# C-bowman/inference-tools

Measured on AMD Instinct MI355X. Metric: GpRegressor fit+predict wall-time and GFLOP/s at N=16384, d=8; % fp64 MFMA peak, higher is better.
Workload: dtype f64

## Files before the change

inference-tools_amd/csrc/api.hip:

```cpp
#include "api_internal.h"
#include <malloc.h>


thread_local std::string g_create_err;


int lane_streams(gpmi_ctx* c, Lane& L) {
  const size_t index = c->lanes.size() - 1;
  L.owns_stream = index < 2;
  if (!L.owns_stream) L.stream = c->lanes[index % 2].stream;
  if (L.owns_stream) HIPCHK(c, hipStreamCreateWithFlags(&L.stream, hipStreamNonBlocking));
  hipDeviceProp_t prop;
  HIPCHK(c, hipGetDeviceProperties(&prop, c->device));
  c->ncu = prop.multiProcessorCount;
  HIPCHK(c, hipEventCreateWithFlags(&L.ev_la, hipEventDisableTiming));
  HIPCHK(c, hipEventCreateWithFlags(&L.ev_panel, hipEventDisableTiming));
  HIPCHK(c, hipEventCreateWithFlags(&L.ev_join, hipEventDisableTiming));
  HIPCHK(c, hipEventCreateWithFlags(&L.ev_main, hipEventDisableTiming));
  HIPCHK(c, hipEventCreateWithFlags(&L.ev_slice, hipEventDisableTiming));
  return GPMI_OK;
}


bool ensure_masked_pair(gpmi_ctx* c, Lane& L, int k) {
// ... 305 lines not shown
  L.early.ident = early_identity;
  L.early.ident_ld = c->ld;
  L.identity_ready = false;
  if (!early_fill) L.early.pending = false;
  potrf_lower(c, L, L.A, c->np, c->ld, L.invD, L.info + slot, allow_lookahead);
  if (!early_fill) L.early.pending = true;
  lane_run_early(L, s);
  if (prebuild_inv2 && L.su[0] && c->np >= 4 * GPMI_OB) {
    HIPCHK(c, hipEventRecord(L.ev_join, s));
    HIPCHK(c, hipStreamWaitEvent(L.su[0], L.ev_join, 0));
    if (int rc = ensure_inv2(c, L, L.su[0])) return rc;
    HIPCHK(c, hipEventRecord(L.ev_main, L.su[0]));
  }
  trsv_forward(c, s, L.A, c->np, c->ld, L.invD, L.vec + 2 * c->np, L.vec, L.info + slot, BatchShape(), true);
  if (prebuild_inv2 && L.inv2_valid && L.su[0]) {
    HIPCHK(c, hipEventRecord(L.ev_la, s));
    HIPCHK(c, hipStreamWaitEvent(L.su[0], L.ev_la, 0));
    launch_lml_reduce(L.su[0], L.vec, L.A, c->ld, c->np, L.red + 2 * slot);
    HIPCHK(c, hipEventRecord(L.ev_main, L.su[0]));
  } else {
    launch_lml_reduce(s, L.vec, L.A, c->ld, c->np, L.red + 2 * slot);
  }
  HIPCHK(c, hipGetLastError());
  return GPMI_OK;
}

int ensure_second_matrix(gpmi_ctx* c, Lane& L) {
  if (!L.B2) HIPCHK(c, hipMalloc(&L.B2, sizeof(double) * c->np * c->ld));
  return GPMI_OK;
}

int ensure_inv2(gpmi_ctx* c, Lane& F, hipStream_t s) {
  if (F.inv2_valid) return GPMI_OK;
  const int64_t nob = (c->np / GPMI_NB + 3) / 4;
  if (!F.inv2) HIPCHK(c, hipMalloc(&F.inv2, sizeof(double) * nob * GPMI_OB * GPMI_OB));
  if (!F.inv2_t) HIPCHK(c, hipMalloc(&F.inv2_t, sizeof(double) * nob * 256 * 256));
  build_inv2(s, F.A, c->np, c->ld, F.invD, F.inv2, F.inv2_t);
  HIPCHK(c, hipGetLastError());
  F.inv2_valid = true;
  return GPMI_OK;
}

int ensure_trsm_panel(gpmi_ctx* c, int64_t rows) {
  if (rows <= c->trsm_panel_rows) return GPMI_OK;
  if (c->trsm_panel) (void)hipFree(c->trsm_panel);
  c->trsm_panel = nullptr;
  c->trsm_panel_rows = 0;
  HIPCHK(c, hipMalloc(&c->trsm_panel, sizeof(double) * rows * (GPMI_OB + 32)));
  c->trsm_panel_rows = rows;
  return GPMI_OK;
}

int enqueue_inverse_factor(gpmi_ctx* c, Lane& L, Lane& F) {
  if (int rc = ensure_inv2(c, F, L.stream)) return rc;
  if (int rc = ensure_trsm_panel(c, c->np)) return rc;
  if (!L.identity_ready) launch_set_identity(L.stream, L.B2, c->ld, c->np);
  L.identity_ready = false;
  trsm_rows_forward(c, L.stream, F.A, c->np, c->ld, F.inv2, L.B2, c->np, true, nullptr, c->trsm_panel);
  return GPMI_OK;
}

int ensure_batch_ws(gpmi_ctx* c, int want) {
  const int64_t per = c->np * c->ld * (int64_t)sizeof(double);
  static const int64_t budget_gib = [] {
    const char* e = std::getenv("GPMI_BATCH_GIB");
    const int v = e ? std::atoi(e) : 24;
    return (int64_t)(v >= 1 && v <= 200 ? v : 24);
  }();
  static const int max_chunk = [] {
    const char* e = std::getenv("GPMI_BATCH_MAX");
    const int v = e ? std::atoi(e) : 512;
    return v >= 2 && v <= 4096 ? v : 512;
  }();
  int cap = (int)((budget_gib << 30) / per);
  if (cap > max_chunk) cap = max_chunk;
  if (cap < 1) cap = 1;
  if (want > cap) want = cap;
  if (want <= c->bcap) return GPMI_OK;
  ARGCHK(c, c->bpend[0] == 0 && c->bpend[1] == 0,
         "the batch workspace cannot grow while an asynchronous batch is pending (gpmi_lml_batch_wait first)");
  auto fr = [](double*& p) {
// ... 569 lines not shown
```

inference-tools_amd/csrc/api_linv.hip:

```cpp
#include "api_internal.h"

void linv_free(LinvState& S) {
  for (double** p : {&S.A, &S.At, &S.y, &S.sig2, &S.zero, &S.K, &S.T, &S.J, &S.J2, &S.Q, &S.X, &S.invD, &S.inv2,
                     &S.inv2_t, &S.panel, &S.vec, &S.gws}) {
    if (*p) (void)hipFree(*p);
    *p = nullptr;
  }
  S = LinvState();
}

namespace {

__global__ void linv_add_diag_kernel(double* __restrict__ J, int64_t ld, const double* __restrict__ sig2,
                                     int64_t mp) {
  const int64_t i = (int64_t)blockIdx.x * blockDim.x + threadIdx.x;
  if (i < mp) J[i * ld + i] += sig2[i];
}


int linv_alloc(gpmi_ctx* c, double** p, int64_t doubles) {
  if (*p) return GPMI_OK;
  HIPCHK(c, hipMalloc(p, sizeof(double) * doubles));
  ZERO_SYNC(c, *p, sizeof(double) * doubles);
  return GPMI_OK;
// ... 95 lines not shown
  *lml = -0.5 * L.h_red[0] - L.h_red[1];
  INFOCHK(c, L.h_info[0]);
  if (info) *info = L.h_info[0];
  return GPMI_OK;
}

int gpmi_linv_lml(gpmi_ctx* c, int kernel, const double* theta, int n_theta, double extra_diag,
                  const double* mu, double* lml, int* info) {
  if (!c) return GPMI_ERR_ARG;
  if (int rc = linv_ready(c)) return rc;
  KParams p;
  if (int rc = make_params(c, kernel, theta, n_theta, extra_diag, p)) return rc;
  return linv_lml_impl(c, p, nullptr, mu, lml, info);
}

int gpmi_linv_lml_dense(gpmi_ctx* c, const double* K_host, const double* mu, double* lml, int* info) {
  if (!c) return GPMI_ERR_ARG;
  if (int rc = linv_ready(c)) return rc;
  ARGCHK(c, K_host, "K is NULL");
  return linv_lml_impl(c, KParams{}, K_host, mu, lml, info);
}

static int linv_lml_grad_impl(gpmi_ctx* c, const KParams& p, int n_theta, const double* K_host, const double* mu,
                              double* lml, double* grad_theta, double* trace_q, double* G_host, double* at_alpha,
                              int* info) {
  ARGCHK(c, mu && lml && (grad_theta || G_host), "mu / lml / output is NULL");
  if (int rc = set_device(c)) return rc;
  LinvState& S = c->linv;
  Lane& L = c->lanes[0];
  hipStream_t s = L.stream;
  const int nt = (int)(c->np / GPMI_NB), mt = (int)(S.mp / GPMI_NB);
  const int64_t vmax = S.mp > c->np ? S.mp : c->np;
  if (int rc = linv_alloc(c, &S.J2, S.mp * S.ldm)) return rc;
  if (int rc = linv_alloc(c, &S.inv2, (int64_t)((mt + 3) / 4) * GPMI_OB * GPMI_OB)) return rc;
  if (int rc = linv_alloc(c, &S.inv2_t, (int64_t)((mt + 3) / 4) * 256 * 256)) return rc;
  if (int rc = linv_alloc(c, &S.panel, S.mp * (GPMI_OB + 32))) return rc;
  const int64_t need = n_theta >= 0 ? grad_ws_doubles(c->np, n_theta) : 0;
  if (S.gws_doubles < need) {
    if (S.gws) (void)hipFree(S.gws);
    S.gws = nullptr;
    S.gws_doubles = 0;
    HIPCHK(c, hipMalloc(&S.gws, sizeof(double) * need));
    S.gws_doubles = need;
  }
  if (int rc = linv_factor(c, p, mu, K_host)) return rc;
  double* v = S.vec;
  double* alpha = S.vec + 4 * vmax;
  double* w = S.vec + 5 * vmax;
  double* gout = L.red + 16;
  trsv_backward(c, s, S.J, S.mp, S.ldm, S.invD, v, alpha, L.info);
  launch_rows_dot(s, S.At, S.ldm, c->np, S.mp, alpha, w);
  build_inv2(s, S.J, S.mp, S.ldm, S.invD, S.inv2, S.inv2_t);
  launch_set_identity(s, S.J2, S.ldm, S.mp);
  trsm_rows_forward(c, s, S.J, S.mp, S.ldm, S.inv2, S.J2, S.mp, true, nullptr, S.panel);
  launch_gemm(s, TILES_LOWER, OP_ASSIGN, false, 1, S.J, S.ldm, S.J2, S.ldm, S.J2, S.ldm, mt, mt, (int)S.mp);
  launch_mirror_lower(s, S.J, S.ldm, S.mp);
  launch_gemm_nt(s, TILES_RECT, OP_ASSIGN, S.T, c->ld, S.J, S.ldm, S.At, S.ldm, mt, nt, (int)S.mp);
  launch_gemm(s, TILES_RECT, OP_ASSIGN, true, 0, S.K, c->ld, S.At, S.ldm, S.T, c->ld, nt, nt, (int)S.mp);
  if (n_theta >= 0) launch_lml_grad(s, p, n_theta, c->x, c->n, c->np, S.K, c->ld, w, w, S.gws, gout);
  HIPCHK(c, hipGetLastError());
  HIPCHK(c, hipMemcpyAsync(L.h_red, L.red, 2 * sizeof(double), hipMemcpyDeviceToHost, s));
  if (n_theta >= 0)
    HIPCHK(c, hipMemcpyAsync(L.h_red + 16, gout, sizeof(double) * (n_theta + 1), hipMemcpyDeviceToHost, s));
  if (G_host)
    HIPCHK(c, hipMemcpy2DAsync(G_host, sizeof(double) * c->n, S.K, sizeof(double) * c->ld, sizeof(double) * c->n, c->n,
                               hipMemcpyDeviceToHost, s));
  HIPCHK(c, hipMemcpyAsync(L.h_info, L.info, sizeof(int), hipMemcpyDeviceToHost, s));
  if (at_alpha) HIPCHK(c, hipMemcpyAsync(at_alpha, w, sizeof(double) * c->n, hipMemcpyDeviceToHost, s));
  HIPCHK(c, hipStreamSynchronize(s));
// ... 6 lines not shown
  return GPMI_OK;
}

int gpmi_linv_lml_grad(gpmi_ctx* c, int kernel, const double* theta, int n_theta, double extra_diag,
                       const double* mu, double* lml, double* grad_theta, double* trace_q,
                       double* at_alpha, int* info) {
  if (!c) return GPMI_ERR_ARG;
  if (int rc = linv_ready(c)) return rc;
  KParams p;
  if (int rc = make_params(c, kernel, theta, n_theta, extra_diag, p)) return rc;
  ARGCHK(c, grad_theta, "grad_theta is NULL");
  return linv_lml_grad_impl(c, p, n_theta, nullptr, mu, lml, grad_theta, trace_q, nullptr, at_alpha, info);
}

int gpmi_linv_lml_grad_dense(gpmi_ctx* c, const double* K_host, const double* mu, double* lml, double* G_host,
                             double* at_alpha, int* info) {
  if (!c) return GPMI_ERR_ARG;
  if (int rc = linv_ready(c)) return rc;
  ARGCHK(c, K_host && G_host, "K / G is NULL");
  return linv_lml_grad_impl(c, KParams{}, -1, K_host, mu, lml, nullptr, nullptr, G_host, at_alpha, info);
}

static int linv_posterior_impl(gpmi_ctx* c, const KParams& p, const double* K_host, const double* mu, double* mean,
                               double* cov, int* info) {
  ARGCHK(c, mu && mean, "mu / mean is NULL");
  if (int rc = set_device(c)) return rc;
  LinvState& S = c->linv;
  Lane& L = c->lanes[0];
  hipStream_t s = L.stream;
  const int nt = (int)(c->np / GPMI_NB), mt = (int)(S.mp / GPMI_NB);
  const int64_t vmax = S.mp > c->np ? S.mp : c->np;
  if (int rc = linv_alloc(c, &S.Q, c->np * S.ldm)) return rc;
  if (int rc = linv_alloc(c, &S.X, c->np * S.ldm)) return rc;
  if (int rc = linv_alloc(c, &S.inv2, (int64_t)((mt + 3) / 4) * GPMI_OB * GPMI_OB)) return rc;
  if (int rc = linv_alloc(c, &S.inv2_t, (int64_t)((mt + 3) / 4) * 256 * 256)) return rc;
  if (int rc = linv_factor(c, p, mu, K_host)) return rc;
  double* v = S.vec;
  double* dm = S.vec + 5 * vmax;
  build_inv2(s, S.J, S.mp, S.ldm, S.invD, S.inv2, S.inv2_t);
  launch_gemm_nt(s, TILES_RECT, OP_ASSIGN, S.Q, S.ldm, S.K, c->ld, S.A, c->ld, nt, mt, (int)c->np);
  trsm_rows_forward(c, s, S.J, S.mp, S.ldm, S.inv2, S.Q, c->np, false, S.X, nullptr);
  launch_rows_dot(s, S.X, S.ldm, c->np, S.mp, v, dm);
  if (cov) launch_gemm_nt(s, TILES_RECT, OP_SUB, S.K, c->ld, S.X, S.ldm, S.X, S.ldm, nt, nt, (int)S.mp);
  HIPCHK(c, hipGetLastError());
  HIPCHK(c, hipMemcpyAsync(L.h_info, L.info, sizeof(int), hipMemcpyDeviceToHost, s));
  HIPCHK(c, hipMemcpyAsync(mean, dm, sizeof(double) * c->n, hipMemcpyDeviceToHost, s));
  if (cov)
    HIPCHK(c, hipMemcpy2DAsync(cov, sizeof(double) * c->n, S.K, sizeof(double) * c->ld, sizeof(double) * c->n,
                               c->n, hipMemcpyDeviceToHost, s));
  HIPCHK(c, hipStreamSynchronize(s));
  c->fitted = false;
  for (int64_t i = 0; i < c->n; ++i) mean[i] += mu[i];
  INFOCHK(c, L.h_info[0]);
  if (info) *info = L.h_info[0];
  return GPMI_OK;
}

int gpmi_linv_posterior(gpmi_ctx* c, int kernel, const double* theta, int n_theta, double extra_diag,
                        const double* mu, double* mean, double* cov, int* info) {
  if (!c) return GPMI_ERR_ARG;
  if (int rc = linv_ready(c)) return rc;
  KParams p;
  if (int rc = make_params(c, kernel, theta, n_theta, extra_diag, p)) return rc;
  return linv_posterior_impl(c, p, nullptr, mu, mean, cov, info);
}

int gpmi_linv_posterior_dense(gpmi_ctx* c, const double* K_host, const double* mu, double* mean, double* cov,
                              int* info) {
// ... 9 lines not shown
```

inference-tools_amd/csrc/gemm_f64.hip:

```cpp
#include <cstdlib>

#include "gemm_tiles.h"

namespace {

using namespace gemm_tiles;

struct GemmArgs {
  double* C;
  const double* A;
  const double* B;
  int64_t ldc, lda, ldb;
  int ntr, ntc, k;
  int kskip;
  unsigned long long* stamp;
  int64_t sC, sA, sB;
  int split, tile_base;
  FlowHook hook;
  int zlocal_tiles;
  int mixed_full;
};

struct WgId {
  int wid;
// ... 237 lines not shown
                      int64_t ldc, const double* A, int64_t lda, const double* B, int64_t ldb, int ntr,
                      int ntc, int k, unsigned long long* stamp, const GemmBatch& bt, int part, int64_t nfull,
                      int64_t nend = -1) {
  if (ntr <= 0 || ntc <= 0 || k <= 0) return;
  if (tiles == TILES_LOWER && ntc > ntr) ntc = ntr;
  const int64_t big = (tiles == TILES_RECT) ? (int64_t)ntr * ntc
                                            : (int64_t)ntc * (ntc + 1) / 2 + (int64_t)(ntr - ntc) * ntc;
  int bm = 128, bn = 128;
  static const int64_t BIG_MIN = [] {
    const char* e = std::getenv("GPMI_BIG_MIN");
    return (int64_t)(e ? std::atoi(e) : 384);
  }();
  static const int64_t SMALL_M32_MAX = [] {
    const char* e = std::getenv("GPMI_M32_MAX");
    return (int64_t)(e ? std::atoi(e) : 192);
  }();
  const int64_t m32_max = bt.ncu_hint > 0 ? SMALL_M32_MAX * bt.ncu_hint / 256 : SMALL_M32_MAX;
  const bool small = part == 0 && ((k <= 128) || (big * bt.count < BIG_MIN));
  if (part == 2) {
    bm = 64;
    bn = 64;
  } else if (small && kskip != 1) {
    if (ntc == 1 && tiles == TILES_RECT && op == OP_ASSIGN) {
      bm = (!b_kmajor && (int64_t)ntr * 2 * bt.count <= m32_max) ? 32 : 64;
    } else if (!b_kmajor || op == OP_SUB) {
      bm = 64;
      bn = 64;
      if (tiles == TILES_RECT && !b_kmajor && k > 128 && big * 4 * bt.count <= m32_max && !bt.ring_order_only) bm = 32;
      static const bool bn32 = [] {
        const char* e = std::getenv("GPMI_CHAIN_BN32");
        return !e || std::atoi(e) != 0;
      }();
      if (bn32 && bm == 32 && kskip == 2 && op == OP_ASSIGN && big * 8 * bt.count <= 2 * 256) bn = 32;
    }
  }
  if (part == 0 && kskip == 4 && b_kmajor && op == OP_ASSIGN && tiles == TILES_RECT) {
    if (big * 16 * bt.count <= 2 * 256) {
      bm = 32;
      bn = 32;
    } else {
      bm = 64;
      bn = 128;
    }
  }
  if (bt.b_lower_tri && kskip == 0 && bn == 128 && bm <= 64 && ntc == 1 && k == 128 && !b_kmajor && op == OP_ASSIGN) kskip = 3;
  GemmArgs g{C, A, B, ldc, lda, ldb, ntr * (128 / bm), ntc * (128 / bn), k, kskip, stamp,
             bt.sC, bt.sA, bt.sB, part == 2 ? 1 : 0, (part == 2 || part == 3) ? (int)nfull : 0, bt.hook, 0, 0};
  int64_t nwg;
  if (tiles == TILES_RECT)
    nwg = (int64_t)g.ntr * g.ntc;
  else
    nwg = (int64_t)g.ntc * (g.ntc + 1) / 2 + (int64_t)(g.ntr - g.ntc) * g.ntc;
  if (part == 1) nwg = nfull;
  if (nend < 0 || nend > big) nend = big;
  if (part == 2) nwg = 4 * (nend - nfull);
  if (part == 3) nwg = nend - nfull;
  if (part == 4) {
    g.mixed_full = (int)nfull;
    nwg = nfull + 4 * (nend - nfull);
  }
  if (nwg <= 0) return;
  dim3 grid((unsigned)nwg, 1, (unsigned)bt.count), block(256);
  static const bool batch_xcd = [] {
    const char* e = std::getenv("GPMI_BATCH_XCD");
    return !e || std::atoi(e) != 0;
  }();
// ... 61 lines not shown
    if (b_kmajor) GPMI_LAUNCH(TILES_RECT, OP_ASSIGN, 1, 32, 32); else GPMI_LAUNCH(TILES_RECT, OP_ASSIGN, 0, 32, 32);
  } else if (bm == 32) {
    if (op == OP_SUB) GPMI_LAUNCH(TILES_RECT, OP_SUB, 0, 32, 64); else GPMI_LAUNCH(TILES_RECT, OP_ASSIGN, 0, 32, 64);
  } else {
    if (tiles == TILES_RECT) {
      if (op == OP_SUB) {
        if (b_kmajor) GPMI_LAUNCH(TILES_RECT, OP_SUB, 1, 64, 64); else GPMI_LAUNCH(TILES_RECT, OP_SUB, 0, 64, 64);
      } else {
        GPMI_LAUNCH(TILES_RECT, OP_ASSIGN, 0, 64, 64);
      }
    } else {
      if (op == OP_SUB) GPMI_LAUNCH(TILES_LOWER, OP_SUB, 0, 64, 64); else GPMI_LAUNCH(TILES_LOWER, OP_ASSIGN, 0, 64, 64);
    }
  }
#undef GPMI_LAUNCH
}
}

void launch_gemm(hipStream_t s, GemmTiles tiles, GemmOp op, bool b_kmajor, int kskip, double* C,
                 int64_t ldc, const double* A, int64_t lda, const double* B, int64_t ldb, int ntr,
                 int ntc, int k, unsigned long long* stamp, const GemmBatch& bt) {
  launch_gemm_part(s, tiles, op, b_kmajor, kskip, C, ldc, A, lda, B, ldb, ntr, ntc, k, stamp, bt, 0, 0);
}

int64_t gemm_split_point(int64_t T, int ncu, int k) {
  static const int64_t BIG_MIN = [] {
    const char* e = std::getenv("GPMI_BIG_MIN");
    return (int64_t)(e ? std::atoi(e) : 384);
  }();
  static const int64_t SPLIT_PCT = [] {
    const char* e = std::getenv("GPMI_SPLIT_PCT");
    return (int64_t)(e ? std::atoi(e) : 70);
  }();
  if (k <= 128 || T < BIG_MIN || ncu <= 0) return T;
  const int64_t rem = T % ncu;
  if (rem == 0 || rem * 100 > (int64_t)ncu * SPLIT_PCT) return T;
  return T - rem;
}

bool gemm_mixed_launches() {
  static const bool mixed = [] {
    const char* e = std::getenv("GPMI_GEMM_MIXED");
    return !e || std::atoi(e) != 0;
  }();
  return mixed;
}

void launch_gemm_nt_split(hipStream_t s, GemmTiles tiles, GemmOp op, double* C, int64_t ldc, const double* A,
                          int64_t lda, const double* B, int64_t ldb, int ntr, int ntc, int k, int64_t nfull,
                          unsigned long long* stamp, unsigned long long* stamp_rest, int64_t nend) {
  if (tiles == TILES_LOWER && ntc > ntr) ntc = ntr;
  const int64_t T = (tiles == TILES_RECT) ? (int64_t)ntr * ntc
                                          : (int64_t)ntc * (ntc + 1) / 2 + (int64_t)(ntr - ntc) * ntc;
  const GemmBatch one{};
  if (nend < 0 || nend > T) nend = T;
  if (nfull >= T) {
    launch_gemm_part(s, tiles, op, false, 0, C, ldc, A, lda, B, ldb, ntr, ntc, k, stamp, one, 0, 0);
    return;
  }
  if (gemm_mixed_launches() && nfull > 0 && nend > nfull && k % 128 == 0 && k > 128) {
    launch_gemm_part(s, tiles, op, false, 0, C, ldc, A, lda, B, ldb, ntr, ntc, k, stamp, one, 4, nfull, nend);
    return;
  }
  launch_gemm_part(s, tiles, op, false, 0, C, ldc, A, lda, B, ldb, ntr, ntc, k, stamp, one, 1, nfull);
  if (nend > nfull)
    launch_gemm_part(s, tiles, op, false, 0, C, ldc, A, lda, B, ldb, ntr, ntc, k, stamp_rest, one, 2, nfull, nend);
}

void launch_gemm_nt_range(hipStream_t s, GemmTiles tiles, GemmOp op, double* C, int64_t ldc, const double* A,
// ... 13 lines not shown
```

inference-tools_amd/csrc/gpmi_internal.h:

```cpp
#pragma once
#include <hip/hip_runtime.h>
#include <cstdint>
#include <string>
#include <vector>

#include "gpmi.h"

constexpr int GPMI_NB = 128;
constexpr int GPMI_MAX_D = 64;
constexpr int GPMI_INFO_FLOW_TIMEOUT = -6;
constexpr int GPMI_NPAIRS = 1;

typedef double d2_t __attribute__((ext_vector_type(2)));
typedef double d4_t __attribute__((ext_vector_type(4)));

static inline int64_t round_up(int64_t v, int64_t m) { return (v + m - 1) / m * m; }

struct KParams {
  int kernel;
  int d;
  double a2;
  double kappa;
  double extra_diag;
  double inv_l2[GPMI_MAX_D];
// ... 263 lines not shown

void launch_gemm(hipStream_t s, GemmTiles tiles, GemmOp op, bool b_kmajor, int kskip, double* C,
                 int64_t ldc, const double* A, int64_t lda, const double* B, int64_t ldb, int ntr,
                 int ntc, int k, unsigned long long* stamp = nullptr, const GemmBatch& bt = GemmBatch());

hipStream_t potrf_first_update_stream(gpmi_ctx* c, Lane& lane, int64_t np, bool allow_lookahead);
void potrf_pair_quiesce(Lane& lane);
void launch_potrf_diag(hipStream_t s, double* Ablk, int64_t ld, double* invD, int* info, int col0,
                       unsigned long long* dbg = nullptr, const BatchShape& bs = BatchShape(), int* pub = nullptr,
                       int pub_val = 0);
void launch_potrf_diag_fault(hipStream_t s, double* Ablk, int64_t ld, const BatchShape& bs = BatchShape());
void potrf_lower_batched(gpmi_ctx* c, hipStream_t s, double* A, int64_t np, int64_t ld, double* invD,
                         int* info, const BatchShape& bs);
void launch_kbuild_square_batched(hipStream_t s, int kernel, const KParams* pdev, int batch, const double* x,
                                  int64_t n, int64_t np, const double* noise, double* A, int64_t ld,
                                  int64_t stride, int d, int64_t noise_stride = 0);
void potrf_lower(gpmi_ctx* c, Lane& lane, double* A, int64_t np, int64_t ld, double* invD,
                 int* info, bool allow_lookahead = true);

bool potrf_flow_enabled(gpmi_ctx* c, Lane& lane, int m);
bool potrf_flow_tail(gpmi_ctx* c, Lane& lane, double* A, int64_t ld, double* invD, int* info, int nt, int t0);
void potrf_flow_free(Lane& lane);

void trsv_forward(gpmi_ctx* c, hipStream_t s, const double* L, int64_t np, int64_t ld,
                  const double* invD, const double* r, double* out, int* err = nullptr,
                  const BatchShape& bs = BatchShape(), bool prefilled = false);
void trsv_backward(gpmi_ctx* c, hipStream_t s, const double* L, int64_t np, int64_t ld,
                   const double* invD, const double* r, double* out, int* err = nullptr,
                   const BatchShape& bs = BatchShape(), bool prefilled = false);
void lane_run_early(Lane& lane, hipStream_t s);
void trsm_identity_batched(hipStream_t s, const double* L, int64_t np, int64_t ld, const double* invD, double* Q,
                           const BatchShape& bs);
constexpr int GPMI_OB = 512;
void build_inv2(hipStream_t s, const double* L, int64_t np, int64_t ld, const double* invD, double* inv2,
                double* tmp);
void trsm_rows_forward(gpmi_ctx* c, hipStream_t s, const double* L, int64_t np, int64_t ld,
                       const double* inv2, double* Q, int64_t mp, bool upper_rhs, double* Qout,
                       double* panel);
void launch_set_identity(hipStream_t s, double* Q, int64_t ld, int64_t np, int batch = 1, int64_t sMat = 0);
void launch_copy(hipStream_t s, const double* src, double* dst, int64_t n);
void launch_copy_rows(hipStream_t s, const double* src, int64_t spitch, double* dst, int64_t dpitch, int64_t width,
                      int64_t height);
void launch_residual(hipStream_t s, const double* y, const double* mu, double mu_const, double* r,
                     int64_t n, int64_t np);
void launch_residual_batched(hipStream_t s, const double* y, const double* mus, const double* mu_consts,
                             double* r, int64_t n, int64_t np, const BatchShape& bs);
void launch_lml_reduce(hipStream_t s, const double* v, const double* L, int64_t ld, int64_t np,
                       double* red, const BatchShape& bs = BatchShape());
void launch_rows_dot(hipStream_t s, const double* Q, int64_t ld, int64_t mp, int64_t np,
                     const double* a, double* out, int batch = 1, int64_t sQ = 0, int64_t sVec = 0);
void launch_rows_sumsq(hipStream_t s, const double* Q, int64_t ld, int64_t mp, int64_t np,
                       double base, double* out, int batch = 1, int64_t sQ = 0, int64_t sVec = 0, double sign = 1.0);

void trsm_rows_backward(gpmi_ctx* c, hipStream_t s, const double* L, int64_t np, int64_t ld,
                        const double* invD, double* Q, int64_t mp, const double* inv2 = nullptr, double* panel = nullptr);

void launch_sd_reduce(hipStream_t s, const KParams& p, const double* x, int64_t n, const double* pts,
                      int64_t m, const double* Kq, int64_t ld, const double* W, int64_t ldw,
                      double scale, double* out);
void launch_grad_rhs(hipStream_t s, const KParams& p, const double* x, int64_t n, int64_t np,
                     const double* pts, int64_t rows_valid, int64_t rows_padded, const double* Kq,
                     int64_t ld, double* G);
void launch_grad_cov(hipStream_t s, const KParams& p, const double* G, int64_t ld, int64_t np,
                     int64_t m, double* cov);
```

inference-tools_amd/csrc/solve.hip:

```cpp
#include <cstdlib>
#include <mutex>

#include "gpmi_internal.h"

namespace {

constexpr int NB = GPMI_NB;

__device__ inline double wave_sum(double v) {
#pragma unroll
  for (int off = 32; off > 0; off >>= 1) v += __shfl_down(v, off, 64);
  return v;
}

constexpr unsigned long long FLOW_SENTINEL = 0xFFF8DEADBEEF0000ull;
constexpr int FLOW_THREADS = 512;
constexpr int FLOW_SPIN_LIMIT = 1 << 22;

__device__ inline double flow_poll(const double* p, int* err, bool& dead) {
  const unsigned long long* q = reinterpret_cast<const unsigned long long*>(p);
  unsigned long long bits = __hip_atomic_load(q, __ATOMIC_RELAXED, __HIP_MEMORY_SCOPE_AGENT);
  int spins = 0;
  while (bits == FLOW_SENTINEL && !dead) {
    __builtin_amdgcn_s_sleep(1);
// ... 215 lines not shown
#pragma unroll
      for (int i = 0; i < 8; ++i) {
        const double x = aj[wave + 64 + 8 * i];
        acc[0] = fma(hb[i][0], x, acc[0]);
        acc[1] = fma(hb[i][1], x, acc[1]);
      }
    }
  }
  part[wave][2 * lane] = acc[0];
  part[wave][2 * lane + 1] = acc[1];
  __syncthreads();
  SWEEP_STAMP(2, step);
  if (tid < NB) {
    double s = 0.0;
#pragma unroll
    for (int g = 0; g < 8; ++g) s += part[g][tid];
    u[tid] = wk - s;
  }
  __syncthreads();
  SWEEP_STAMP(3, step);
  {
    double s = 0.0;
#pragma unroll
    for (int i = 0; i < 32; ++i) s = fma(xi[i], u[rg * 32 + i], s);
    part[4 + rg][col] = s;
    __syncthreads();
    if (tid < NB)
      flow_publish(a + (int64_t)k * NB + tid, (part[4][tid] + part[5][tid]) + (part[6][tid] + part[7][tid]));
    SWEEP_STAMP(4, step);
    SWEEP_STAMP_FLUSH(step);
  }
}

__global__ void inv2_seed_kernel(const double* __restrict__ invD, double* __restrict__ inv2, int nt) {
  const int b = blockIdx.z, r = blockIdx.y, cpair = (blockIdx.x * 64 + threadIdx.x) * 2;
  const int t = r >> 7;
  d2_t v = d2_t{0.0, 0.0};
  if ((cpair >> 7) == t && 4 * b + t < nt)
    v = *reinterpret_cast<const d2_t*>(invD + ((int64_t)(4 * b + t) * NB + (r & 127)) * NB + (cpair & 127));
  *reinterpret_cast<d2_t*>(inv2 + ((int64_t)b * GPMI_OB + r) * GPMI_OB + cpair) = v;
}

__global__ void copy_panel_kernel(const double* __restrict__ src, int64_t lds, double* __restrict__ dst,
                                  int64_t ldd) {
  const int64_t r = blockIdx.y;
  const int c = (blockIdx.x * 64 + threadIdx.x) * 2;
  *reinterpret_cast<d2_t*>(dst + r * ldd + c) = *reinterpret_cast<const d2_t*>(src + r * lds + c);
}

__global__ void set_identity_kernel(double* __restrict__ Q, int64_t ld, int64_t np, int64_t sMat) {
  const int64_t j = ((int64_t)blockIdx.x * blockDim.x + threadIdx.x) * 2;
  const int64_t i = blockIdx.y;
  Q += (int64_t)blockIdx.z * sMat;
  if (j < np)
    *reinterpret_cast<d2_t*>(Q + i * ld + j) = d2_t{j == i ? 1.0 : 0.0, j + 1 == i ? 1.0 : 0.0};
}

__global__ void copy_rows_kernel(const double* __restrict__ src, int64_t spitch, double* __restrict__ dst, int64_t dpitch,
                                 int64_t width) {
  const int64_t j = (int64_t)blockIdx.x * blockDim.x + threadIdx.x;
  if (j < width) dst[(int64_t)blockIdx.y * dpitch + j] = src[(int64_t)blockIdx.y * spitch + j];
}

__global__ void copy_kernel(const double* __restrict__ src, double* __restrict__ dst, int64_t n) {
  const int64_t i = (int64_t)blockIdx.x * blockDim.x + threadIdx.x;
  if (i < n) dst[i] = src[i];
}

__global__ void residual_batched_kernel(const double* __restrict__ y, const double* __restrict__ mus,
                                        const double* __restrict__ mu_consts, double* __restrict__ r,
                                        int64_t n, int64_t np, int64_t sVec) {
  const int64_t i = (int64_t)blockIdx.x * blockDim.x + threadIdx.x;
  if (i >= np) return;
// ... 123 lines not shown
    launch_set_identity(s, e.ident, e.ident_ld, e.np);
    lane.identity_ready = true;
  }
}

void trsv_forward(gpmi_ctx* c, hipStream_t s, const double* L, int64_t np, int64_t ld,
                  const double* invD, const double* r, double* out, int* err, const BatchShape& bs, bool prefilled) {
  const int nt = (int)(np / NB);
  flow_gate_enter(c, s, (int64_t)nt);
  ProfScope ps(c, s, GPMI_PROF_SOLVE, (double)np * np, 4.0 * np * np);
  if (!prefilled)
    hipLaunchKernelGGL(flow_fill_kernel, dim3((unsigned)((np + 255) / 256), 1, (unsigned)bs.count), dim3(256), 0, s,
                       out, np, bs.sVec);
  const unsigned grid = bs.count > 1 ? 8u * (unsigned)nt * (unsigned)((bs.count + 7) / 8) : (unsigned)nt;
  hipLaunchKernelGGL(trsv_fwd_flow_kernel, dim3(grid), dim3(FLOW_THREADS), 0, s, L, ld, invD, r, out, err, bs.sMat,
                     bs.sInv, bs.sVec, nt, bs.count);
  flow_gate_leave(c, s, (int64_t)nt);
}

void trsv_backward(gpmi_ctx* c, hipStream_t s, const double* L, int64_t np, int64_t ld,
                   const double* invD, const double* r, double* out, int* err, const BatchShape& bs, bool prefilled) {
  const int nt = (int)(np / NB);
  flow_gate_enter(c, s, (int64_t)nt);
  ProfScope ps(c, s, GPMI_PROF_SOLVE, (double)np * np, 4.0 * np * np);
  if (!prefilled)
    hipLaunchKernelGGL(flow_fill_kernel, dim3((unsigned)((np + 255) / 256), 1, (unsigned)bs.count), dim3(256), 0, s, out,
                       np, bs.sVec);
  const unsigned grid = bs.count > 1 ? 8u * (unsigned)nt * (unsigned)((bs.count + 7) / 8) : (unsigned)nt;
  hipLaunchKernelGGL(trsv_bwd_flow_kernel, dim3(grid), dim3(FLOW_THREADS), 0, s, L, ld, invD, r, out, err, nt, bs.sMat,
                     bs.sInv, bs.sVec, bs.count);
  flow_gate_leave(c, s, (int64_t)nt);
}

void build_inv2(hipStream_t s, const double* L, int64_t np, int64_t ld, const double* invD, double* inv2,
                double* tmp) {
  const int nt = (int)(np / NB);
  const int nob = (nt + 3) / 4;
  const int64_t slot = (int64_t)GPMI_OB * GPMI_OB, tslot = 256 * 256;
  hipLaunchKernelGGL(inv2_seed_kernel, dim3(GPMI_OB / 2 / 64, GPMI_OB, (unsigned)nob), dim3(64), 0, s, invD, inv2,
                     nt);
  auto offdiag = [&](int r0, int c0, int h2, int h1, int count) {
    if (count <= 0 || h2 <= 0) return;
    const GemmBatch b1{count, tslot, 4 * NB * ld + 4 * NB, slot};
    launch_gemm(s, TILES_RECT, OP_ASSIGN, true, 0, tmp, 256, L + (int64_t)r0 * NB * ld + (int64_t)c0 * NB, ld,
                inv2 + (int64_t)c0 * NB * GPMI_OB + (int64_t)c0 * NB, GPMI_OB, h2, h1, h1 * NB, nullptr, b1);
    const GemmBatch b2{count, slot, slot, tslot};
    launch_gemm(s, TILES_RECT, OP_SUB, true, 0, inv2 + (int64_t)r0 * NB * GPMI_OB + (int64_t)c0 * NB, GPMI_OB,
                inv2 + (int64_t)r0 * NB * GPMI_OB + (int64_t)r0 * NB, GPMI_OB, tmp, 256, h2, h1, h2 * NB, nullptr,
                b2);
  };
  offdiag(1, 0, 1, 1, (nt - 1 + 3) / 4);
  offdiag(3, 2, 1, 1, (nt - 3 + 3) / 4);
  const int full = nt / 4;
  offdiag(2, 0, 2, 2, full);
  if (nt % 4 == 3) {
    const int64_t b = full;
    const GemmBatch one{};
    const double* Lb = L + (b * 4 * NB) * ld + b * 4 * NB;
    double* Xb = inv2 + b * slot;
    double* Tb = tmp + b * tslot;
    launch_gemm(s, TILES_RECT, OP_ASSIGN, true, 0, Tb, 256, Lb + (int64_t)2 * NB * ld, ld, Xb, GPMI_OB, 1, 2, 2 * NB,
                nullptr, one);
    launch_gemm(s, TILES_RECT, OP_SUB, true, 0, Xb + (int64_t)2 * NB * GPMI_OB, GPMI_OB,
                Xb + (int64_t)2 * NB * GPMI_OB + 2 * NB, GPMI_OB, Tb, 256, 1, 2, NB, nullptr, one);
  }
}

void trsm_rows_forward(gpmi_ctx* c, hipStream_t s, const double* L, int64_t np, int64_t ld,
                       const double* inv2, double* Q, int64_t mp, bool upper_rhs, double* Qout,
                       double* panel) {
  const int nt = (int)(np / NB), mt_all = (int)(mp / NB);
  const int OBT = GPMI_OB / NB;
  const int64_t ldp = GPMI_OB + 32;
  ProfScope ps(c, s, GPMI_PROF_TRSM, (double)mp * np * np, 4.0 * np * np);
  for (int J = 0; J < nt; J += OBT) {
    const int Je = (J + OBT < nt) ? J + OBT : nt;
    const int w = Je - J;
    const int mt = upper_rhs ? (Je < mt_all ? Je : mt_all) : mt_all;
    double* QJ = Q + (int64_t)J * NB;
    double* X = Qout ? Qout + (int64_t)J * NB : panel;
    const int64_t ldx = Qout ? ld : ldp;
    launch_gemm(s, TILES_RECT, OP_ASSIGN, false, 2, X, ldx, QJ, ld, inv2 + (int64_t)(J / OBT) * GPMI_OB * GPMI_OB,
                GPMI_OB, mt, w, w * NB);
    const int rest = nt - Je;
    if (rest > 0)
      launch_gemm_nt_split(s, TILES_RECT, OP_SUB, Q + (int64_t)Je * NB, ld, X, ldx,
                           L + (int64_t)Je * NB * ld + (int64_t)J * NB, ld, mt, rest, w * NB,
                           gemm_split_point((int64_t)mt * rest, c->ncu, w * NB));
    if (!Qout) {
      const int64_t rows = (int64_t)mt * NB;
      hipLaunchKernelGGL(copy_panel_kernel, dim3((unsigned)(w * NB / 2 / 64), (unsigned)rows), dim3(64), 0, s, panel,
                         ldp, QJ, ld);
    }
  }
}

void trsm_rows_backward(gpmi_ctx* c, hipStream_t s, const double* L, int64_t np, int64_t ld,
                        const double* invD, double* Q, int64_t mp, const double* inv2, double* panel) {
  const int nt = (int)(np / NB), mt = (int)(mp / NB);
  ProfScope ps(c, s, GPMI_PROF_TRSM, (double)mp * np * np, 4.0 * np * np);
  static const bool wide = [] {
    const char* e = std::getenv("GPMI_BACKWARD_OB");
    return !e || std::atoi(e) != 0;
  }();
  if (wide && inv2 && panel) {
    const int OBT = GPMI_OB / NB;
    const int64_t ldp = GPMI_OB + 32;
    const int nob = (nt + OBT - 1) / OBT;
    for (int b = nob - 1; b >= 0; --b) {
      const int J = b * OBT, Je = (J + OBT < nt) ? J + OBT : nt, w = Je - J;
      double* QJ = Q + (int64_t)J * NB;
      launch_gemm(s, TILES_RECT, OP_ASSIGN, true, 4, panel, ldp, QJ, ld, inv2 + (int64_t)b * GPMI_OB * GPMI_OB, GPMI_OB, mt, w,
                  w * NB);
      if (J > 0)
        launch_gemm(s, TILES_RECT, OP_SUB, true, 0, Q, ld, panel, ldp, L + (int64_t)J * NB * ld, ld, mt, J, w * NB);
      hipLaunchKernelGGL(copy_panel_kernel, dim3((unsigned)(w * NB / 2 / 64), (unsigned)((int64_t)mt * NB)), dim3(64), 0, s, panel,
                         ldp, QJ, ld);
    }
    return;
  }
  for (int k = nt - 1; k >= 0; --k) {
    double* Qk = Q + (int64_t)k * NB;
    launch_gemm(s, TILES_RECT, OP_ASSIGN, true, false, Qk, ld, Qk, ld, invD + (int64_t)k * NB * NB,
                NB, mt, 1, NB);
    if (k > 0)
      launch_gemm(s, TILES_RECT, OP_SUB, true, false, Q, ld, Qk, ld, L + (int64_t)k * NB * ld, ld, mt,
                  k, NB);
  }
}

void launch_set_identity(hipStream_t s, double* Q, int64_t ld, int64_t np, int batch, int64_t sMat) {
  dim3 grid((unsigned)((np / 2 + 255) / 256), (unsigned)np, (unsigned)batch);
  hipLaunchKernelGGL(set_identity_kernel, grid, dim3(256), 0, s, Q, ld, np, sMat);
}

void trsm_identity_batched(hipStream_t s, const double* L, int64_t np, int64_t ld, const double* invD, double* Q,
                           const BatchShape& bs) {
  const int nt = (int)(np / NB);
  const int OBT = 4;
  launch_set_identity(s, Q, ld, np, bs.count, bs.sMat);
  GemmBatch inplace{bs.count, bs.sMat, bs.sMat, bs.sInv};
  inplace.b_lower_tri = true;
  GemmBatch upd{bs.count, bs.sMat, bs.sMat, bs.sMat};
  upd.ring_order_only = true;
  for (int J = 0; J < nt; J += OBT) {
    const int Je = (J + OBT < nt) ? J + OBT : nt;
// ... 58 lines not shown
```

Measured before the change: 55120.

## Widen forward TRSM inverse-block width to 1024 with recursive inv2 build

```diff
diff --git a/inference-tools_amd/csrc/api.hip b/inference-tools_amd/csrc/api.hip
--- a/inference-tools_amd/csrc/api.hip
+++ b/inference-tools_amd/csrc/api.hip
@@ -361,9 +361,8 @@
 
 int ensure_inv2(gpmi_ctx* c, Lane& F, hipStream_t s) {
   if (F.inv2_valid) return GPMI_OK;
-  const int64_t nob = (c->np / GPMI_NB + 3) / 4;
-  if (!F.inv2) HIPCHK(c, hipMalloc(&F.inv2, sizeof(double) * nob * GPMI_OB * GPMI_OB));
-  if (!F.inv2_t) HIPCHK(c, hipMalloc(&F.inv2_t, sizeof(double) * nob * 256 * 256));
+  if (!F.inv2) HIPCHK(c, hipMalloc(&F.inv2, sizeof(double) * inv2_doubles(c->np)));
+  if (!F.inv2_t) HIPCHK(c, hipMalloc(&F.inv2_t, sizeof(double) * inv2_tmp_doubles(c->np)));
   build_inv2(s, F.A, c->np, c->ld, F.invD, F.inv2, F.inv2_t);
   HIPCHK(c, hipGetLastError());
   F.inv2_valid = true;
@@ -375,7 +374,7 @@
   if (c->trsm_panel) (void)hipFree(c->trsm_panel);
   c->trsm_panel = nullptr;
   c->trsm_panel_rows = 0;
-  HIPCHK(c, hipMalloc(&c->trsm_panel, sizeof(double) * rows * (GPMI_OB + 32)));
+  HIPCHK(c, hipMalloc(&c->trsm_panel, sizeof(double) * rows * (predict_ob() + 32)));
   c->trsm_panel_rows = rows;
   return GPMI_OK;
 }
diff --git a/inference-tools_amd/csrc/api_linv.hip b/inference-tools_amd/csrc/api_linv.hip
--- a/inference-tools_amd/csrc/api_linv.hip
+++ b/inference-tools_amd/csrc/api_linv.hip
@@ -151,9 +151,9 @@
   const int nt = (int)(c->np / GPMI_NB), mt = (int)(S.mp / GPMI_NB);
   const int64_t vmax = S.mp > c->np ? S.mp : c->np;
   if (int rc = linv_alloc(c, &S.J2, S.mp * S.ldm)) return rc;
-  if (int rc = linv_alloc(c, &S.inv2, (int64_t)((mt + 3) / 4) * GPMI_OB * GPMI_OB)) return rc;
-  if (int rc = linv_alloc(c, &S.inv2_t, (int64_t)((mt + 3) / 4) * 256 * 256)) return rc;
-  if (int rc = linv_alloc(c, &S.panel, S.mp * (GPMI_OB + 32))) return rc;
+  if (int rc = linv_alloc(c, &S.inv2, inv2_doubles(S.mp))) return rc;
+  if (int rc = linv_alloc(c, &S.inv2_t, inv2_tmp_doubles(S.mp))) return rc;
+  if (int rc = linv_alloc(c, &S.panel, S.mp * (predict_ob() + 32))) return rc;
   const int64_t need = n_theta >= 0 ? grad_ws_doubles(c->np, n_theta) : 0;
   if (S.gws_doubles < need) {
     if (S.gws) (void)hipFree(S.gws);
@@ -226,8 +226,8 @@
   const int64_t vmax = S.mp > c->np ? S.mp : c->np;
   if (int rc = linv_alloc(c, &S.Q, c->np * S.ldm)) return rc;
   if (int rc = linv_alloc(c, &S.X, c->np * S.ldm)) return rc;
-  if (int rc = linv_alloc(c, &S.inv2, (int64_t)((mt + 3) / 4) * GPMI_OB * GPMI_OB)) return rc;
-  if (int rc = linv_alloc(c, &S.inv2_t, (int64_t)((mt + 3) / 4) * 256 * 256)) return rc;
+  if (int rc = linv_alloc(c, &S.inv2, inv2_doubles(S.mp))) return rc;
+  if (int rc = linv_alloc(c, &S.inv2_t, inv2_tmp_doubles(S.mp))) return rc;
   if (int rc = linv_factor(c, p, mu, K_host)) return rc;
   double* v = S.vec;
   double* dm = S.vec + 5 * vmax;
diff --git a/inference-tools_amd/csrc/gemm_f64.hip b/inference-tools_amd/csrc/gemm_f64.hip
--- a/inference-tools_amd/csrc/gemm_f64.hip
+++ b/inference-tools_amd/csrc/gemm_f64.hip
@@ -293,6 +293,15 @@
         return !e || std::atoi(e) != 0;
       }();
       if (bn32 && bm == 32 && kskip == 2 && op == OP_ASSIGN && big * 8 * bt.count <= 2 * 256) bn = 32;
+      static const int wide_wgs = [] {
+        const char* e = std::getenv("GPMI_WIDE_CHAIN_WGS");
+        return e ? std::atoi(e) : 4;
+      }();
+      if (bn32 && tiles == TILES_RECT && !b_kmajor && kskip == 2 && op == OP_ASSIGN && k > GPMI_OB && bt.count == 1 &&
+          !bt.ring_order_only && big * 16 <= (int64_t)wide_wgs * 256) {
+        bm = 32;
+        bn = 32;
+      }
     }
   }
   if (part == 0 && kskip == 4 && b_kmajor && op == OP_ASSIGN && tiles == TILES_RECT) {
@@ -420,9 +429,13 @@
     const char* e = std::getenv("GPMI_SPLIT_PCT");
     return (int64_t)(e ? std::atoi(e) : 70);
   }();
+  static const int64_t SPLIT_PCT_WIDE = [] {
+    const char* e = std::getenv("GPMI_SPLIT_PCT_WIDE");
+    return (int64_t)(e ? std::atoi(e) : 100);
+  }();
   if (k <= 128 || T < BIG_MIN || ncu <= 0) return T;
   const int64_t rem = T % ncu;
-  if (rem == 0 || rem * 100 > (int64_t)ncu * SPLIT_PCT) return T;
+  if (rem == 0 || rem * 100 > (int64_t)ncu * (k > GPMI_OB ? SPLIT_PCT_WIDE : SPLIT_PCT)) return T;
   return T - rem;
 }
 
diff --git a/inference-tools_amd/csrc/gpmi_internal.h b/inference-tools_amd/csrc/gpmi_internal.h
--- a/inference-tools_amd/csrc/gpmi_internal.h
+++ b/inference-tools_amd/csrc/gpmi_internal.h
@@ -319,6 +319,10 @@
 void trsm_identity_batched(hipStream_t s, const double* L, int64_t np, int64_t ld, const double* invD, double* Q,
                            const BatchShape& bs);
 constexpr int GPMI_OB = 512;
+int predict_ob();
+int64_t inv2_doubles(int64_t np);
+int64_t inv2_tmp_doubles(int64_t np);
+const double* inv2_block512(const double* inv2, int b);
 void build_inv2(hipStream_t s, const double* L, int64_t np, int64_t ld, const double* invD, double* inv2,
                 double* tmp);
 void trsm_rows_forward(gpmi_ctx* c, hipStream_t s, const double* L, int64_t np, int64_t ld,
diff --git a/inference-tools_amd/csrc/solve.hip b/inference-tools_amd/csrc/solve.hip
--- a/inference-tools_amd/csrc/solve.hip
+++ b/inference-tools_amd/csrc/solve.hip
@@ -271,13 +271,13 @@
   }
 }
 
-__global__ void inv2_seed_kernel(const double* __restrict__ invD, double* __restrict__ inv2, int nt) {
+__global__ void inv2_seed_kernel(const double* __restrict__ invD, double* __restrict__ inv2, int nt, int pob) {
   const int b = blockIdx.z, r = blockIdx.y, cpair = (blockIdx.x * 64 + threadIdx.x) * 2;
-  const int t = r >> 7;
+  const int t = r >> 7, T = pob >> 7;
   d2_t v = d2_t{0.0, 0.0};
-  if ((cpair >> 7) == t && 4 * b + t < nt)
-    v = *reinterpret_cast<const d2_t*>(invD + ((int64_t)(4 * b + t) * NB + (r & 127)) * NB + (cpair & 127));
-  *reinterpret_cast<d2_t*>(inv2 + ((int64_t)b * GPMI_OB + r) * GPMI_OB + cpair) = v;
+  if ((cpair >> 7) == t && T * b + t < nt)
+    v = *reinterpret_cast<const d2_t*>(invD + ((int64_t)(T * b + t) * NB + (r & 127)) * NB + (cpair & 127));
+  *reinterpret_cast<d2_t*>(inv2 + ((int64_t)b * pob + r) * pob + cpair) = v;
 }
 
 __global__ void copy_panel_kernel(const double* __restrict__ src, int64_t lds, double* __restrict__ dst,
@@ -467,37 +467,56 @@
   flow_gate_leave(c, s, (int64_t)nt);
 }
 
+int predict_ob() {
+  static const int ob = [] {
+    const char* e = std::getenv("GPMI_PREDICT_OB");
+    const int v = e ? std::atoi(e) : 1024;
+    return (v == GPMI_OB || v == 2048) ? v : 1024;
+  }();
+  return ob;
+}
+
+int64_t inv2_doubles(int64_t np) {
+  const int pob = predict_ob(), T = pob / NB;
+  return (int64_t)((np / NB + T - 1) / T) * pob * pob;
+}
+
+int64_t inv2_tmp_doubles(int64_t np) {
+  const int pob = predict_ob(), T = pob / NB;
+  return (int64_t)((np / NB + T - 1) / T) * (pob / 2) * (pob / 2);
+}
+
+const double* inv2_block512(const double* inv2, int b) {
+  const int pob = predict_ob(), r = pob / GPMI_OB;
+  return inv2 + (int64_t)(b / r) * pob * pob + (int64_t)(b % r) * GPMI_OB * (pob + 1);
+}
+
 void build_inv2(hipStream_t s, const double* L, int64_t np, int64_t ld, const double* invD, double* inv2,
                 double* tmp) {
+  const int pob = predict_ob(), T = pob / NB;
   const int nt = (int)(np / NB);
-  const int nob = (nt + 3) / 4;
-  const int64_t slot = (int64_t)GPMI_OB * GPMI_OB, tslot = 256 * 256;
-  hipLaunchKernelGGL(inv2_seed_kernel, dim3(GPMI_OB / 2 / 64, GPMI_OB, (unsigned)nob), dim3(64), 0, s, invD, inv2,
-                     nt);
-  auto offdiag = [&](int r0, int c0, int h2, int h1, int count) {
-    if (count <= 0 || h2 <= 0) return;
-    const GemmBatch b1{count, tslot, 4 * NB * ld + 4 * NB, slot};
-    launch_gemm(s, TILES_RECT, OP_ASSIGN, true, 0, tmp, 256, L + (int64_t)r0 * NB * ld + (int64_t)c0 * NB, ld,
-                inv2 + (int64_t)c0 * NB * GPMI_OB + (int64_t)c0 * NB, GPMI_OB, h2, h1, h1 * NB, nullptr, b1);
-    const GemmBatch b2{count, slot, slot, tslot};
-    launch_gemm(s, TILES_RECT, OP_SUB, true, 0, inv2 + (int64_t)r0 * NB * GPMI_OB + (int64_t)c0 * NB, GPMI_OB,
-                inv2 + (int64_t)r0 * NB * GPMI_OB + (int64_t)r0 * NB, GPMI_OB, tmp, 256, h2, h1, h2 * NB, nullptr,
-                b2);
-  };
-  offdiag(1, 0, 1, 1, (nt - 1 + 3) / 4);
-  offdiag(3, 2, 1, 1, (nt - 3 + 3) / 4);
-  const int full = nt / 4;
-  offdiag(2, 0, 2, 2, full);
-  if (nt % 4 == 3) {
-    const int64_t b = full;
-    const GemmBatch one{};
-    const double* Lb = L + (b * 4 * NB) * ld + b * 4 * NB;
-    double* Xb = inv2 + b * slot;
-    double* Tb = tmp + b * tslot;
-    launch_gemm(s, TILES_RECT, OP_ASSIGN, true, 0, Tb, 256, Lb + (int64_t)2 * NB * ld, ld, Xb, GPMI_OB, 1, 2, 2 * NB,
-                nullptr, one);
-    launch_gemm(s, TILES_RECT, OP_SUB, true, 0, Xb + (int64_t)2 * NB * GPMI_OB, GPMI_OB,
-                Xb + (int64_t)2 * NB * GPMI_OB + 2 * NB, GPMI_OB, Tb, 256, 1, 2, NB, nullptr, one);
+  const int nslot = (nt + T - 1) / T;
+  const int64_t slot = (int64_t)pob * pob, slotL = (int64_t)T * NB * (ld + 1);
+  hipLaunchKernelGGL(inv2_seed_kernel, dim3(pob / 2 / 64, pob, (unsigned)nslot), dim3(64), 0, s, invD, inv2, nt, pob);
+  for (int hb = 1; hb < T; hb *= 2) {
+    const int64_t tld = (int64_t)hb * NB, tslot = tld * tld;
+    auto offdiag = [&](int s0, int r0, int c0, int h2, int count) {
+      if (count <= 0 || h2 <= 0) return;
+      double* X = inv2 + (int64_t)s0 * slot;
+      const double* Lp = L + (int64_t)s0 * T * NB * (ld + 1);
+      const GemmBatch b1{count, tslot, slotL, slot};
+      launch_gemm(s, TILES_RECT, OP_ASSIGN, true, 0, tmp, tld, Lp + (int64_t)r0 * NB * ld + (int64_t)c0 * NB, ld,
+                  X + (int64_t)c0 * NB * pob + (int64_t)c0 * NB, pob, h2, hb, hb * NB, nullptr, b1);
+      const GemmBatch b2{count, slot, slot, tslot};
+      launch_gemm(s, TILES_RECT, OP_SUB, true, 0, X + (int64_t)r0 * NB * pob + (int64_t)c0 * NB, pob,
+                  X + (int64_t)r0 * NB * pob + (int64_t)r0 * NB, pob, tmp, tld, h2, hb, h2 * NB, nullptr, b2);
+    };
+    for (int c0 = 0; c0 < T; c0 += 2 * hb) {
+      const int r0 = c0 + hb;
+      const int full = nt >= r0 + hb ? (nt - r0 - hb) / T + 1 : 0;
+      offdiag(0, r0, c0, hb, full);
+      if (full < nslot) offdiag(full, r0, c0, nt - (full * T + r0), 1);
+    }
   }
 }
 
@@ -505,8 +524,9 @@
                        const double* inv2, double* Q, int64_t mp, bool upper_rhs, double* Qout,
                        double* panel) {
   const int nt = (int)(np / NB), mt_all = (int)(mp / NB);
-  const int OBT = GPMI_OB / NB;
-  const int64_t ldp = GPMI_OB + 32;
+  const int pob = predict_ob();
+  const int OBT = pob / NB;
+  const int64_t ldp = pob + 32;
   ProfScope ps(c, s, GPMI_PROF_TRSM, (double)mp * np * np, 4.0 * np * np);
   for (int J = 0; J < nt; J += OBT) {
     const int Je = (J + OBT < nt) ? J + OBT : nt;
@@ -515,8 +535,8 @@
     double* QJ = Q + (int64_t)J * NB;
     double* X = Qout ? Qout + (int64_t)J * NB : panel;
     const int64_t ldx = Qout ? ld : ldp;
-    launch_gemm(s, TILES_RECT, OP_ASSIGN, false, 2, X, ldx, QJ, ld, inv2 + (int64_t)(J / OBT) * GPMI_OB * GPMI_OB,
-                GPMI_OB, mt, w, w * NB);
+    launch_gemm(s, TILES_RECT, OP_ASSIGN, false, 2, X, ldx, QJ, ld, inv2 + (int64_t)(J / OBT) * pob * pob, pob, mt, w,
+                w * NB);
     const int rest = nt - Je;
     if (rest > 0)
       launch_gemm_nt_split(s, TILES_RECT, OP_SUB, Q + (int64_t)Je * NB, ld, X, ldx,
@@ -545,8 +565,7 @@
     for (int b = nob - 1; b >= 0; --b) {
       const int J = b * OBT, Je = (J + OBT < nt) ? J + OBT : nt, w = Je - J;
       double* QJ = Q + (int64_t)J * NB;
-      launch_gemm(s, TILES_RECT, OP_ASSIGN, true, 4, panel, ldp, QJ, ld, inv2 + (int64_t)b * GPMI_OB * GPMI_OB, GPMI_OB, mt, w,
-                  w * NB);
+      launch_gemm(s, TILES_RECT, OP_ASSIGN, true, 4, panel, ldp, QJ, ld, inv2_block512(inv2, b), predict_ob(), mt, w, w * NB);
       if (J > 0)
         launch_gemm(s, TILES_RECT, OP_SUB, true, 0, Q, ld, panel, ldp, L + (int64_t)J * NB * ld, ld, mt, J, w * NB);
       hipLaunchKernelGGL(copy_panel_kernel, dim3((unsigned)(w * NB / 2 / 64), (unsigned)((int64_t)mt * NB)), dim3(64), 0, s, panel,
```

New measurement: 55820 (median of 6 runs). 1.3% higher.
